# bjack205/rsLQR

Hardware: AMD Instinct MI355X
Metric: LQR solves/sec (nx=12,nu=4,N=256,batch=1024 per GPU) (higher is better)
Workload: dtype f64; 1 GPU; nx=12 nu=4 N=256 batch=1024 per GPU, fp64, factor+solve per step; parallelism=batch-sharded x1, no data-path collective, ranks_seen=1, flags=0, schedule=reduced-fused2

## Files before the change

include/ndlqr_hip.h:

```cpp
#ifndef NDLQR_HIP_H_
#define NDLQR_HIP_H_

#include <stddef.h>
#include <stdint.h>

#ifdef __cplusplus
extern "C" {
#endif

typedef struct NdlqrHipCtx NdlqrHipCtx;

int ndlqr_hip_device_count(void);
const char* ndlqr_hip_last_error(void);

NdlqrHipCtx* ndlqr_hip_create(int nstates, int ninputs, int nhorizon, int batch, int device);
#define NDLQR_CREATE_NO_PAD 1u
NdlqrHipCtx* ndlqr_hip_create_ex(int nstates, int ninputs, int nhorizon, int batch, int device, unsigned create_flags);
void ndlqr_hip_destroy(NdlqrHipCtx* ctx);
int ndlqr_hip_set_flags(NdlqrHipCtx* ctx, unsigned flags);
unsigned ndlqr_hip_get_flags(const NdlqrHipCtx* ctx);
int ndlqr_hip_set_stream(NdlqrHipCtx* ctx, void* hip_stream);
void* ndlqr_hip_get_stream(NdlqrHipCtx* ctx);

int ndlqr_hip_upload_inputs(NdlqrHipCtx* ctx, int p0, int count, const double* AB,
// ... 73 lines not shown
int ndlqr_hip_solve_polished_adjoint(NdlqrHipCtx* ctx, const double* g, int max_steps, int* steps, int* status);
int ndlqr_hip_download_polish_codes(NdlqrHipCtx* ctx, unsigned char* codes);
int ndlqr_hip_solve_multi_rhs(NdlqrHipCtx* ctx, int nrhs, const double* q, const double* r, const double* d,
                              const double* x0, double* soln);
int ndlqr_hip_solve_multi_rhs_slices(NdlqrHipCtx* ctx, int nrhs, const double* q, const double* r, const double* d,
                                     const double* x0, int knot0, int nknots, unsigned blocks, double* out);

int ndlqr_hip_step_async(NdlqrHipCtx* ctx, const double* q, const double* r, const double* d, const double* x0,
                         double* soln);
int ndlqr_hip_synchronize_previous(NdlqrHipCtx* ctx);
int ndlqr_hip_set_step_selection(NdlqrHipCtx* ctx, int knot0, int nknots, unsigned blocks);
int ndlqr_hip_solve_slices_async(NdlqrHipCtx* ctx, int knot0, int nknots, unsigned blocks, double* out);
int ndlqr_hip_download_selection(NdlqrHipCtx* ctx, int knot0, int nknots, unsigned blocks, double* out);
int ndlqr_hip_time_shard_top_doubles(NdlqrHipCtx* ctx, int G);
int ndlqr_hip_time_shard_factor(NdlqrHipCtx* ctx, int g, int G);
int ndlqr_hip_time_shard_export(NdlqrHipCtx* ctx, int G, double* buf);
int ndlqr_hip_time_shard_import(NdlqrHipCtx* ctx, int G, const double* buf);
int ndlqr_hip_time_shard_finish(NdlqrHipCtx* ctx, int g, int G);
void* ndlqr_hip_host_alloc(size_t bytes);
void ndlqr_hip_host_free(void* p);
void* ndlqr_hip_device_alloc(size_t bytes);
void ndlqr_hip_device_free(void* p);
int ndlqr_hip_copy(void* dst, const void* src, size_t bytes);

int ndlqr_hip_download_solutions(NdlqrHipCtx* ctx, int p0, int count, double* soln);
int ndlqr_hip_download_rhs_blocks(NdlqrHipCtx* ctx, int p, double* z_full);
int ndlqr_hip_download_factors(NdlqrHipCtx* ctx, int p, double* fact);
int ndlqr_hip_factors_valid(const NdlqrHipCtx* ctx);
int ndlqr_hip_pack_solutions_device(NdlqrHipCtx* ctx, double* dst);
int ndlqr_hip_kkt_residual(NdlqrHipCtx* ctx, double* res, double* bnorm);
int ndlqr_hip_cholesky_failures(NdlqrHipCtx* ctx);
const char* ndlqr_hip_schedule(const NdlqrHipCtx* ctx);
int ndlqr_hip_compact_level1(const NdlqrHipCtx* ctx);

int ndlqr_hip_profile_slots(NdlqrHipCtx* ctx);
int ndlqr_hip_profile_get(NdlqrHipCtx* ctx, int slot, char* name, int name_cap, double* total_ms,
                          int* launches);
int ndlqr_hip_profile_reset(NdlqrHipCtx* ctx);

int ndlqr_hip_gemm(int tA, int tB, int m, int n, int k, double alpha, const double* A, int lda,
                   const double* B, int ldb, double beta, double* C, int ldc);
int ndlqr_hip_potrf_lower(int n, double* A, int lda);
int ndlqr_hip_potrs_lower(int n, int nrhs, const double* L, int ldl, double* B, int ldb);
int ndlqr_hip_trsv_lower(int n, int nrhs, const double* L, int ldl, double* B, int ldb, int transposed);

#ifdef __cplusplus
}
#endif
#endif
```

rslqr_amd/api.py:

```python
import ctypes as C
import os
import re

import numpy as np

from . import build as _build

FLAG_STRICT_FP = 1
FLAG_GENERIC = 2
FLAG_PROFILE = 4
FLAG_KEEP_FACT = 8
FLAG_KEEP_RECORDS = 16
SOLN_LAMBDA, SOLN_STATE, SOLN_INPUT, SOLN_ONLY = 1, 2, 4, 8
GRAD_A, GRAD_B, GRAD_Q, GRAD_R, GRAD_q, GRAD_r, GRAD_d, GRAD_x0 = 1, 2, 4, 8, 16, 32, 64, 128
GRAD_NAMES = ("A", "B", "Q", "R", "q", "r", "d", "x0")

ERR_INVALID = -1
ERR_NO_DEVICE = -2
ERR_NOT_SPD = -3

dp = C.POINTER(C.c_double)


class Matrix(C.Structure):
# ... 254 lines not shown
    proto("ndlqr_BatchKktResidualVector", ci, vp, dp)
    proto("ndlqr_hip_refine_phase_ms", ci, vp, dp)
    proto("ndlqr_BatchDeviceContext", vp, vp)
    proto("ndlqr_BatchSetBounds", ci, vp, C.c_uint, dp, dp, dp, dp)
    proto("ndlqr_SolveBatchBoxConstrained", ci, vp, C.POINTER(NdLqrBoxSettingsFull), C.POINTER(ci), C.POINTER(ci))
    proto("ndlqr_CopyBatchBoundMultipliers", ci, vp, dp, dp)
    proto("ndlqr_CopyBatchBoxPenalties", ci, vp, dp)
    proto("ndlqr_CopyBatchBoxResiduals", ci, vp, dp)
    proto("ndlqr_CopyBatchBoxAdjointResiduals", ci, vp, dp)
    proto("ndlqr_BatchSetInfeasibilityDetection", ci, vp, ci, cd)
    proto("ndlqr_CopyBatchInfeasibilityCertificate", ci, vp, dp, dp, dp)
    proto("ndlqr_CopyBatchInfeasibilityMeasures", ci, vp, dp, C.POINTER(ci))
    proto("ndlqr_BatchSetBoxAcceleration", ci, vp, ci, cd, cd)
    proto("ndlqr_CopyBatchBoxAcceleration", ci, vp, C.POINTER(ci), C.POINTER(ci), dp, C.POINTER(ci))
    proto("ndlqr_SolveBatchBoxAdjoint", ci, vp, dp, C.POINTER(NdLqrBoxSettingsFull), C.POINTER(ci), C.POINTER(ci))
    proto("ndlqr_BatchBoundGradients", ci, vp, C.c_uint, dp, dp, dp, dp)
    proto("ndlqr_PolishBatchBoxConstrained", ci, vp, C.POINTER(NdLqrPolishSettings), C.POINTER(ci), C.POINTER(ci))
    proto("ndlqr_hip_download_polish_codes", ci, vp, C.POINTER(C.c_ubyte))
    proto("ndlqr_SolveBatchPolishedAdjoint", ci, vp, dp, C.POINTER(NdLqrPolishSettings), C.POINTER(ci), C.POINTER(ci))
    proto("ndlqr_hip_factor_count", C.c_ulonglong, vp)
    proto("ndlqr_hip_set_stream", ci, vp, vp)
    proto("ndlqr_hip_get_stream", vp, vp)
    proto("ndlqr_hip_profile_slots", ci, vp)
    proto("ndlqr_hip_profile_get", ci, vp, ci, C.c_char_p, ci, dp, C.POINTER(ci))
    proto("ndlqr_hip_profile_reset", ci, vp)
    proto("ndlqr_hip_device_pointers", ci, vp, C.POINTER(vp))
    proto("ndlqr_hip_staged_io", ci, vp, C.POINTER(dp), C.POINTER(dp), C.POINTER(dp), C.POINTER(dp))
    proto("ndlqr_hip_download_rhs_blocks", ci, vp, ci, dp)
    proto("ndlqr_hip_upload_inputs", ci, vp, ci, ci, dp, dp, dp)
    proto("ndlqr_hip_factors_valid", ci, vp)
    proto("ndlqr_hip_schedule", C.c_char_p, vp)
    if hasattr(L, "ndlqr_hip_compact_level1"):
        proto("ndlqr_hip_compact_level1", C.c_int, vp)
    proto("ndlqr_hip_set_pipeline_depth", ci, vp, ci)
    proto("ndlqr_hip_pipeline_depth", ci, vp)
    proto("ndlqr_hip_pack_solutions_device", ci, vp, vp)
    proto("ndlqr_hip_gemm", ci, ci, ci, ci, ci, ci, cd, dp, ci, dp, ci, cd, dp, ci)
    proto("ndlqr_hip_potrf_lower", ci, ci, dp, ci)
    proto("ndlqr_hip_potrs_lower", ci, ci, ci, dp, ci, dp, ci)
    _LIB = L
    return L


def pinned_empty(shape):
    import weakref
    count = int(np.prod(shape))
    L = lib()
    ptr = L.ndlqr_HostAlloc(max(count, 1) * 8)
    if not ptr:
        raise MemoryError("ndlqr_HostAlloc(%d bytes) failed" % (count * 8))
    buf = (C.c_double * max(count, 1)).from_address(ptr)
    arr = np.ctypeslib.as_array(buf)[:count].reshape(shape)
    weakref.finalize(buf, L.ndlqr_HostFree, C.c_void_p(ptr))
    return arr


class DeviceArray:

    def __init__(self, shape):
        import weakref
        self.shape = tuple(int(s) for s in (shape if isinstance(shape, (tuple, list)) else (shape,)))
        self.size = int(np.prod(self.shape))
        L = lib()
        self.ptr = L.ndlqr_DeviceAlloc(max(self.size, 1) * 8)
        if not self.ptr:
            raise MemoryError("ndlqr_DeviceAlloc(%d bytes) failed" % (self.size * 8))
# ... 707 lines not shown
        err = self.L.ndlqr_hip_upload_inputs(self.ctx, 0, self.batch, _ptr(AB), _ptr(QR), _ptr(rhs))
        if err:
            raise RuntimeError("ndlqr_hip_upload_inputs failed: %d" % err)

    def factors(self, p):
        if self.N & (self.N - 1):
            raise RuntimeError("ndlqr_CopyBatchFactors: not available for a padded horizon (horizon %d is no power of two)"
                               % self.N)
        K = int(np.log2(self.N))
        out = np.zeros(self.N * K * (2 * self.n + self.m) * self.n)
        err = self.L.ndlqr_CopyBatchFactors(self.h, p, _ptr(out))
        if err:
            raise RuntimeError("ndlqr_CopyBatchFactors failed: %d" % err)
        return out

    def cholesky_failures(self):
        return self.L.ndlqr_BatchCholeskyFailures(self.h)

    def profile(self):
        out = {}
        for slot in range(self.L.ndlqr_hip_profile_slots(self.ctx)):
            name = C.create_string_buffer(64)
            ms, cnt = C.c_double(0), C.c_int(0)
            self.L.ndlqr_hip_profile_get(self.ctx, slot, name, 64, C.byref(ms), C.byref(cnt))
            out[name.value.decode()] = (ms.value, cnt.value)
        return out

    def schedule(self):
        return self.L.ndlqr_hip_schedule(self.ctx).decode()

    def compact_level1(self):
        return hasattr(self.L, "ndlqr_hip_compact_level1") and bool(self.L.ndlqr_hip_compact_level1(self.ctx))

    def set_pipeline_depth(self, depth):
        return self.L.ndlqr_hip_set_pipeline_depth(self.ctx, depth)

    def pipeline_depth(self):
        return self.L.ndlqr_hip_pipeline_depth(self.ctx)

    def profile_reset(self):
        self.L.ndlqr_hip_profile_reset(self.ctx)
```

rslqr_amd/csrc/hip_context.hpp:

```cpp
#pragma once
#include <hip/hip_runtime.h>

#include <cstdio>
#include <cstdlib>
#include <cstring>
#include <initializer_list>
#include <string>
#include <utility>
#include <vector>

#include "ndlqr.h"
#include "ndlqr_hip.h"

#include "kernels_common.hpp"

#pragma GCC visibility push(hidden)
int ndlqr_hip_fail(const char* what, hipError_t e);
struct NdlqrHipCtx;
int ndlqr_hip_ensure_F(NdlqrHipCtx* c);
#pragma GCC visibility pop
#define HIP_TRY(expr)                                                  \
  do {                                                                 \
    hipError_t e_ = (expr);                                            \
    if (e_ != hipSuccess) return ndlqr_hip_fail(#expr, e_);            \
  } while (0)

constexpr size_t kLdsMax = 160 * 1024;
constexpr size_t kLdsDefaultDynamic = 64 * 1024;
template <class Kernel>
static inline hipError_t allow_dynamic_lds(Kernel* kernel, size_t lds) {
  if (lds <= kLdsDefaultDynamic) return hipSuccess;
  return hipFuncSetAttribute(reinterpret_cast<const void*>(kernel), hipFuncAttributeMaxDynamicSharedMemorySize, (int)lds);
}


enum { SLOT_LEAF = 0, SLOT_SEP, SLOT_SCHUR, SLOT_BOUNDARY, SLOT_APPLY, SLOT_BOTTOM, SLOT_UPPER, SLOT_TOP, SLOT_COUNT };

struct PendingEvent {
  int slot;
  hipEvent_t start, stop;
};

enum class Family { None, Small, GenericReduced, GenericKnot };

struct KeptState {
  Family family = Family::None;
  bool time_shard = false;
  bool rec_complete = false;
  bool rec_compact = false;
  bool fact_valid = false;
  const char* schedule = "none";
  bool rec1_compact = false;
  void forget_factorisation() { rec_complete = fact_valid = false; }
};

struct CapturedChain {
  hipGraphExec_t exec = nullptr;
  unsigned flags = 0;
  hipStream_t stream = nullptr;
  unsigned apply = 0;
  void reset() {
    if (exec) (void)hipGraphExecDestroy(exec);
    exec = nullptr;
  }
};

struct KnotSlice {
  int knot0 = 0, nknots = 0;
  unsigned blocks = 7u;
  bool valid(int N, unsigned allowed) const {
    return knot0 >= 0 && nknots > 0 && knot0 + nknots <= N && (blocks & 7u) && !(blocks & ~allowed);
  }
  size_t width(const ndlqr::Dims& u) const {
    return ((blocks & 1u) ? u.n : 0) + ((blocks & 2u) ? u.n : 0) + ((blocks & 4u) ? u.m : 0);
  }
  size_t doubles(const ndlqr::Dims& u) const { return nknots > 0 ? width(u) * nknots : (size_t)u.rows * u.N - u.m; }
};

#pragma GCC visibility push(hidden)

template <class T, bool PINNED>
class OwnedBuf {
  T* p_ = nullptr;
  size_t n_ = 0;

// ... 37 lines not shown

static inline size_t doubles_QR(const ndlqr::Dims& d) { return (size_t)d.batch * d.N * d.w; }
static inline size_t doubles_z(const ndlqr::Dims& d) { return (size_t)d.batch * d.N * d.rows; }
static inline size_t doubles_F(const ndlqr::Dims& d) { return (size_t)d.batch * d.K * d.N * d.fb; }
static inline hipError_t first_error(std::initializer_list<hipError_t> list) {
  for (const hipError_t e : list) if (e != hipSuccess) return e;
  return hipSuccess;
}

struct BufferSet {
  DevBuf<double> rec;
  DevBuf<double> red;
  DevBuf<double> ytop;
  DevBuf<double> z;
  DevBuf<double> rhs;
  DevBuf<double> xfer;
  DevBuf<int> tree_cnt;
  PinnedBuf<int> h_fail;
  hipStream_t stream = nullptr;
  hipEvent_t ev_start = nullptr, ev_stop = nullptr;
  unsigned long long rhs_gen[4] = {};
  CapturedChain graph;
  bool ready = false;
  hipError_t ensure_xfer(const ndlqr::Dims& u) { return xfer.ensure((size_t)u.batch * u.N * u.rows + (size_t)u.batch * u.n); }
};


struct DevKnobs {
  int rowbcast = -1;
  int tree = -1;
  int backsub_cols = -1;
  int fuse2 = -1;
  int compact1 = -1;
  int pipeline = 2;
  bool no_top = false;
  int top_levels = 3;
  bool no_mfma = false;
  int sep_threads = 0;
  int mult_threads = 0;
  bool no_reduced_generic = false;
  bool no_pad = false;
  bool alt_priority_set = false;
  int alt_priority = 0;
};

struct AdjointState {
  DevBuf<double> rhs, z;
  DevBuf<double> save;
  unsigned long long gen = 0;
  hipError_t ensure_save(const ndlqr::Dims& d) { return save.ensure(2 * (size_t)d.batch * d.N * d.n); }
  hipError_t ensure(const ndlqr::Dims& d, hipStream_t st) {
    return first_error({rhs.ensure(doubles_z(d)), z.ensure_zeroed(doubles_z(d), st), ensure_save(d)});
  }
};

struct BoxState {
  DevBuf<double> lo, hi, v, y, z, qr_save, rhs[2], resid, rho;
  DevBuf<unsigned char> mask;
  DevBuf<int> status, iters, word;
  PinnedBuf<int> h_word;
  bool shared = false, have_bounds = false, have_vy = false;
  size_t bstride = 0;
  bool fact = false;
  bool rho_uniform = false;
  double rho_value = 0.0;
  unsigned flags = 0;
// ... 296 lines not shown
```

rslqr_amd/csrc/kernels_bottom_reduced.hpp:

```cpp
#pragma once
#include "kernels_dpp.hpp"
#include "kernels_small.hpp"

namespace ndlqr {

typedef double acc4_t __attribute__((ext_vector_type(4)));

template <int NX>
struct McPitch {
  static constexpr int SP = 18, WP = 17;
};

template <int NX, class Hook>
__device__ __forceinline__ void factor_tail_mc(const int lane, const acc4_t& c, const double (&ra)[(NX + 3) / 4],
                                               const double (&rb)[(NX + 3) / 4], const double* Wm, acc4_t& X0,
                                               acc4_t& X1, Hook hook) {
  constexpr int KS = (NX + 3) / 4, WP = McPitch<NX>::WP;
  int lane_o = lane;
  asm volatile("" : "+v"(lane_o));
  const int li = lane_o & 15, lk = lane_o >> 4;
  double wt[KS], wa[KS], b0[KS];
#pragma unroll
  for (int q = 0; q < KS; ++q) {
    wt[q] = Wm[(4 * q + lk) * WP + li];
// ... 181 lines not shown
  for (int g = 0; g < 4; ++g) {
    buf[P::SCR_A + (lk + 4 * g) * SP + li] = cA[g];
    buf[P::SCR_B + (lk + 4 * g) * SP + li] = cB[g];
  }
  wave_lds_sync();
  const double* tile = buf + (lk < 2 ? P::SCR_A : P::SCR_B);
  double acc[NX];
  if constexpr (NX % 2 == 0) {
#pragma unroll
    for (int j = 0; j < NX; j += 2) {
      const double2 t = *reinterpret_cast<const double2*>(&tile[ri * SP + j]);
      acc[j] = t.x; acc[j + 1] = t.y;
    }
  } else {
#pragma unroll
    for (int j = 0; j < NX; ++j) acc[j] = tile[ri * SP + j];
  }
  if (h == NX) {
#pragma unroll
    for (int k = 0; k < NX; ++k) w[k] = tile[k * SP + NX];
  }
  const bool bad = rb_chol_inv<NX, false>(li, acc, w);
  wave_lds_sync();
  {
    const int x = lk >> 1;
    double* ydst = buf + (h <= NX ? P::tile(x, 0) + h : P::tile(x, 1) + (h <= 2 * NX ? h - NX - 1 : YP - 1));
#pragma unroll
    for (int k = 0; k < NX; ++k) ydst[k * YP] = w[k];
    if constexpr (4 * KS > NX) {
#pragma unroll
      for (int e0 = 0; e0 < (4 * KS - NX) * YP; e0 += 16) {
        const int e = e0 + li;
        if (e < (4 * KS - NX) * YP) buf[P::tile(x, lk & 1) + NX * YP + e] = 0.0;
      }
    }
  }
  if ((lk & 1) == 0 && li < NX) {
    double* lr = (lk == 0 ? lrecA : lrecB) + li * (li + 1) / 2;
#pragma unroll
    for (int c = 0; c < NX; ++c)
      if (c <= li) lr[c] = acc[c];
  }
  wave_lds_sync();
  return bad;
}

template <int NX, bool N00, bool N01, bool N10, bool N11>
__device__ __forceinline__ void gram_mc(const double (&R0)[(NX + 3) / 4], const double (&R1)[(NX + 3) / 4],
                                        const acc4_t& X0, const acc4_t& X1, acc4_t& g00, acc4_t& g01, acc4_t& g10,
                                        acc4_t& g11) {
  constexpr int KS = (NX + 3) / 4;
  const acc4_t zero = {0.0, 0.0, 0.0, 0.0};
  g00 = zero; g01 = zero; g10 = zero; g11 = zero;
#pragma unroll
  for (int q = 0; q < KS; ++q) {
    if constexpr (N00) g00 = __builtin_amdgcn_mfma_f64_16x16x4f64(R0[q], X0[q], g00, 0, 0, 0);
    if constexpr (N01) g01 = __builtin_amdgcn_mfma_f64_16x16x4f64(R0[q], X1[q], g01, 0, 0, 0);
    if constexpr (N10) g10 = __builtin_amdgcn_mfma_f64_16x16x4f64(R1[q], X0[q], g10, 0, 0, 0);
    if constexpr (N11) g11 = __builtin_amdgcn_mfma_f64_16x16x4f64(R1[q], X1[q], g11, 0, 0, 0);
  }
}

template <int NX> __device__ __forceinline__ constexpr bool rows_all(int g) { return 4 * g + 3 < NX; }
template <int NX> __device__ __forceinline__ constexpr bool rows_none(int g) { return 4 * g >= NX; }

template <int NX>
// ... 300 lines not shown
  constexpr int NN = NX * NX, KS = P::KS;
  const int N = d.N, T = 8, s = base + 3;
  const bool hasA = base > 0, hasB = base + T < N, leftchild = (base & T) == 0;
  const int li = lane & 15, lk = lane >> 4;
  double y0[KS], y1[KS];
  acc4_t Z0 = {0.0, 0.0, 0.0, 0.0}, Z1 = {0.0, 0.0, 0.0, 0.0};
#pragma unroll
  for (int q = 0; q < KS; ++q) {
    y0[q] = buf[P::Y0 + (4 * q + lk) * P::YP + li];
    y1[q] = buf[P::Y1 + (4 * q + lk) * P::YP + li];
    Z0[q] = y0[q]; Z1[q] = y1[q];
  }
  if (gram) {
    const RedSlot<NX> sa = red_slot<NX>(red, d, b, hasA ? base - 1 : s);
    const RedSlot<NX> sb = red_slot<NX>(red, d, b, hasB ? base + T - 1 : s);
    acc4_t g00, g01, g11, unused;
    gram_mc<NX, true, true, false, true>(y0, y1, Z0, Z1, g00, g01, unused, g11);
    const acc4_t zero = {0.0, 0.0, 0.0, 0.0};
    push_mc<NX>(lane, hasA, hasB, leftchild, sa, sb, g00, g01, g11, zero, zero, zero, AddAtomic(), StorePlain());
  } else {
    double wt[KS];
#pragma unroll
    for (int q = 0; q < KS; ++q) wt[q] = buf[P::W + (4 * q + lk) * P::WP + li];
    acc4_t X0 = {0.0, 0.0, 0.0, 0.0}, X1 = {0.0, 0.0, 0.0, 0.0};
#pragma unroll
    for (int q = 0; q < KS; ++q) {
      X0 = __builtin_amdgcn_mfma_f64_16x16x4f64(wt[q], y0[q], X0, 0, 0, 0);
      X1 = __builtin_amdgcn_mfma_f64_16x16x4f64(wt[q], y1[q], X1, 0, 0, 0);
    }
    store_record_mc<NX>(rec + ((size_t)b * N + s) * (2 * NN + NX), lane, hasA, hasB, X0, X1);
  }
}

template <int NX, int NU, bool TREE, bool REDIRECT, bool C1 = false>
__device__ __forceinline__ void bottom_group_mc(const Dims& d, const int k0, const int b, const int lane,
                                                const double* __restrict__ AB, const double* __restrict__ QR,
                                                const double* __restrict__ rhs, double* red, double* __restrict__ rec,
                                                double* F, int* __restrict__ info, const int store_l, const int compact0,
                                                ReducedLds<NX, NU>& lds, double* slotA, double* slotB,
                                                const bool with_m = false, acc4_t* c_m = nullptr);
template <int NX, int NU, bool C1 = false>
__global__ __launch_bounds__(128) __attribute__((amdgpu_waves_per_eu(4))) void bottom8_reduced_mc(
    Dims d, const double* __restrict__ AB, const double* __restrict__ QR, const double* __restrict__ rhs, double* red,
    double* __restrict__ rec, int* __restrict__ info) {
  __shared__ ReducedLds<NX, NU> lds[2];
  __shared__ __attribute__((aligned(16))) double mslot[RedSlot<NX>::SIZE];
  const int wave = __builtin_amdgcn_readfirstlane(threadIdx.x >> 6), b = blockIdx.y;
  const int kw = (blockIdx.x + d.xoff) * 8;
  int lane = threadIdx.x & 63;
  for (int e = threadIdx.x; e < RedSlot<NX>::SIZE; e += 128) mslot[e] = 0.0;
  __syncthreads();
  acc4_t c_m = {0.0, 0.0, 0.0, 0.0};
  bottom_group_mc<NX, NU, false, true, C1>(d, kw + 4 * wave, b, lane, AB, QR, rhs, red, rec, nullptr, info, 0, 1, lds[wave],
                                       wave == 1 ? mslot : nullptr, wave == 0 ? mslot : nullptr, wave == 0, &c_m);
  asm volatile("s_waitcnt vmcnt(0)" ::: "memory");
  __syncthreads();
  asm volatile("" : "+v"(lane));
  if (wave == 0) reduced_eliminate_pass_mc<NX, NU>(d, kw, b, lane, c_m, mslot, info, lds[0].buf);
  __syncthreads();
  reduced_eliminate_tail_mc<NX, NU>(d, kw, b, lane, wave == 0, red, rec, lds[0].buf);
}

template <int NX>
__device__ __forceinline__ void backsub_top_body(const Dims& d, const int b, const int t,
                                                 const double* __restrict__ recs, double* __restrict__ ytop,
                                                 double* ytop_lds, const int bp = -1, const double* zsep = nullptr);
template <int NX, int NU>
__global__ __launch_bounds__(256) __attribute__((amdgpu_waves_per_eu(4))) void reduced_top_mc(Dims d, const int l0, const double* __restrict__ AB,
                                                      const double* __restrict__ QR, const double* __restrict__ rhs,
                                                      double* red, double* __restrict__ rec, double* F,
                                                      int* __restrict__ info, const int store_l,
                                                      double* __restrict__ ytop) {
  __shared__ ReducedLds<NX, NU, false> lds[4];
  const int wave = __builtin_amdgcn_readfirstlane(threadIdx.x >> 6), b = blockIdx.x;
  for (int l = l0, s0 = 0; l < d.K;) {
    int lane = threadIdx.x & 63;
    asm volatile("" : "+v"(lane));
    const int cnt = d.N >> (l + 1);
    if (wave + s0 < cnt)
      reduced_separator_mc<NX, NU, true>(d, l, (wave + s0) * (2 << l), b, lane, AB, QR, rhs, red, rec, F, info, store_l,
                                         lds[wave]);
    s0 += 4;
    if (s0 < cnt) continue;
    s0 = 0;
    ++l;
    asm volatile("s_waitcnt vmcnt(0)" ::: "memory");
    __syncthreads();
  }
  if (ytop) backsub_top_body<NX>(d, b, threadIdx.x, rec, ytop, reinterpret_cast<double*>(&lds[0]), -1, nullptr);
}

template <int NX, int NU, bool TREE, bool REDIRECT, bool C1>
__device__ __forceinline__ void bottom_group_mc(const Dims& d, const int k0, const int b, const int lane,
                                                const double* __restrict__ AB, const double* __restrict__ QR,
                                                const double* __restrict__ rhs, double* red, double* __restrict__ rec,
                                                double* F, int* __restrict__ info, const int store_l, const int compact0,
                                                ReducedLds<NX, NU>& lds, double* slotA, double* slotB,
                                                const bool with_m, acc4_t* c_m) {
  constexpr int W = NX + NU, ROWS = 2 * NX + NU, NN = NX * NX, KSN = (NX + 3) / 4;
  constexpr int REC = 2 * NN + NX;
  constexpr int WP = ReducedLds<NX, NU>::WP;
  double* abs_ = lds.buf;
  double* rq = lds.rq;
  double* rh = lds.rh;
  const int N = d.N;
  const int li = lane & 15, lk = lane >> 4;
  const int ri = li < NX ? li : NX - 1;
  const bool hasA = k0 > 0, hasB = k0 + 4 < N;
  SEG_INIT();

  {
    const double* abm = AB + ((size_t)b * N + k0) * NX * W;
    const double* q0 = QR + ((size_t)b * N + k0) * W;
    const double* r0 = rhs + ((size_t)b * N + k0) * ROWS;
    constexpr int NQ = 4 * W, IQ = (NQ + 63) / 64, NR = 4 * ROWS, IR = (NR + 63) / 64;
    double qv[IQ], rv[IR];
#pragma unroll
    for (int it = 0; it < IQ; ++it) { const int e = lane + 64 * it; qv[it] = q0[e < NQ ? e : NQ - 1]; }
#pragma unroll
    for (int it = 0; it < IR; ++it) { const int e = lane + 64 * it; rv[it] = r0[e < NR ? e : NR - 1]; }
    if constexpr (W % 2 == 0) {
      constexpr int NA = 4 * NX * W / 2, IA = (NA + 63) / 64;
      double2 t[IA];
#pragma unroll
      for (int it = 0; it < IA; ++it) {
        const int e = lane + 64 * it;
        t[it] = reinterpret_cast<const double2*>(abm)[e < NA ? e : NA - 1];
      }
#pragma unroll
      for (int it = 0; it < IA; ++it) {
        const int e = lane + 64 * it, ec = e < NA ? e : NA - 1, row = ec / (W / 2), c2 = ec - row * (W / 2);
// ... 96 lines not shown
        y1[q] = Y1[(4 * q + lk) * PY::YP + li];
        Z0[q] = y0[q]; Z1[q] = y1[q];
      }
      if (x == 0) hook_s0(y0, y1, Z0, Z1); else hook_s2(y0, y1, Z0, Z1);
    }
    SEG(35);
  } else {
  double ra0[KSN], rb0[KSN], ra2[KSN], rb2[KSN];
#pragma unroll
  for (int q = 0; q < KSN; ++q) {
    const int kq = 4 * q + lk, i = kq < NX ? kq : NX - 1;
    const double a0 = abs_[i * WP + ri], b0 = abs_[(NX + ri) * WP + i];
    const double a2 = abs_[(2 * NX + i) * WP + ri], b2 = abs_[(3 * NX + ri) * WP + i];
    const double s0 = rq[ri], s1 = rq[W + i], s2 = rq[2 * W + ri], s3 = rq[3 * W + i];
    ra0[q] = hasA ? -a0 * s0 : 0.0;
    rb0[q] = -b0 * s1;
    ra2[q] = -a2 * s2;
    rb2[q] = hasB ? -b2 * s3 : 0.0;
  }
  wave_lds_sync();
  SEG(21);

  using Pair = McPairLayout<NX>;
  if (chol_pair_mc<NX>(lane, c_s0, c_s2, lds.buf, store_l ? Fblk(F, d, b, 0, k0 + 1) : nullptr,
                       store_l ? Fblk(F, d, b, 0, k0 + 3) : nullptr) &&
      (lane == 0 || lane == 32))
    flag_failure(info, d, b);
  SEG(30);
  factor_tail_mc<NX>(lane, c_s0, ra0, rb0, lds.buf + Pair::W_A, X0, X1, hook_s0);
  store_record_mc<NX>(myrec, lane, hasA, true, X0, X1);
  factor_tail_mc<NX>(lane, c_s2, ra2, rb2, lds.buf + Pair::W_B, X0, X1, hook_s2);
  store_record_mc<NX>(myrec + 2 * REC, lane, true, hasB, X0, X1);
  SEG(35);
  }
  double wcol[NX];
  {
    constexpr int TP = 17;
    static_assert(2 * 16 * TP <= ReducedLds<NX, NU>::NBUF, "both coupling tiles fit the buffer");
    double* ta = lds.buf;
    double* tb = lds.buf + 16 * TP;
    wave_lds_sync();
#pragma unroll
    for (int g = 0; g < 4; ++g) {
      ta[(lk + 4 * g) * TP + li] = -ca_t[g];
      tb[(lk + 4 * g) * TP + li] = -cb_t[g];
    }
    wave_lds_sync();
    const int h = lane & 31;
    const bool is_a = h < NX, is_b = h > NX && h <= 2 * NX;
    const double* src = is_a ? ta + h : tb + (is_b ? h - NX - 1 : 0);
#pragma unroll
    for (int k = 0; k < NX; ++k) wcol[k] = src[k * TP];
    wave_lds_sync();
  }
  const bool leftchild = (k0 & 4) == 0;
  RedSlot<NX> sa = red_slot<NX>(red, d, b, hasA ? k0 - 1 : 3);
  RedSlot<NX> sb = red_slot<NX>(red, d, b, hasB ? k0 + 3 : 3);
  if constexpr (REDIRECT) {
    if (slotA) sa.p = slotA;
    if (slotB) sb.p = slotB;
  }
  if constexpr (C1) {
    static_assert(!TREE, "the tree schedule keeps full records");
    if (chol_pair_y_mc<NX>(lane, c_t, c_t, lds.buf, wcol, myrec + REC, myrec + REC) && lane == 0) flag_failure(info, d, b);
    SEG(34);
    using PY = McPairYLayout<NX>;
// ... 74 lines not shown
```

rslqr_amd/csrc/launch_small.hpp:

```cpp
#pragma once
#include "hip_context.hpp"
#include "kernels_leaf.hpp"
#include "kernels_small.hpp"
#include "kernels_bottom_reduced.hpp"
#include "kernels_rowbcast.hpp"

constexpr int kBottomLevels = 2;

struct SmallPlan {
  bool strict, keep;
  bool lean;
  int store_l;
  bool reduced;
  bool tree;
  bool compact;
  bool rowbcast;
  bool fuse2;
  bool compact1;
  int level0;
  int ltop;
  int top_l0;
  bool top_sweeps;
  size_t top_lds;
  const char* schedule;
  bool rec_complete, rec_compact;
  bool needs_F;
};

template <int NX, int NU>
constexpr bool kRbBacksubFits = 8 * (2 * NX + NU) <= 256;

static inline unsigned apply_grid(const NdlqrHipCtx* c, const ndlqr::Dims& d) {
  return (unsigned)(c->apply_nblk > 0 ? c->apply_nblk : d.N / 8);
}
static inline ndlqr::Dims apply_dims(const NdlqrHipCtx* c, const ndlqr::Dims& d) {
  ndlqr::Dims da = d;
  if (c->apply_nblk > 0) da.xoff += c->apply_blk0;
  return da;
}

template <int NX, int NU>
constexpr bool kCompact1Fits = ndlqr::P1OnMatrixCores<NX, NU>::value && NX >= 9 && NX + NU <= 16;

template <int NX, int NU, bool MULTI, class... Args>
static void launch_rb_backsub(const NdlqrHipCtx* c, const dim3 grid, hipStream_t stream, const bool compact1,
                              const Args&... args) {
  if constexpr (NX + NU <= 16) {
    if constexpr (kCompact1Fits<NX, NU> && !MULTI) {
      if (compact1) {
        hipLaunchKernelGGL((ndlqr::rb_backsub<NX, NU, false, true, true>), grid, dim3(ndlqr::kRbBacksubColsThreads), 0, stream,
                           args...);
        return;
      }
    }
    if (c->knobs.backsub_cols != 0) {
      hipLaunchKernelGGL((ndlqr::rb_backsub<NX, NU, MULTI, true>), grid, dim3(ndlqr::kRbBacksubColsThreads), 0, stream, args...);
      return;
    }
  }
  hipLaunchKernelGGL((ndlqr::rb_backsub<NX, NU, MULTI, false>), grid, dim3(256), 0, stream, args...);
}

template <int NX, int NU>
static SmallPlan plan_small(const NdlqrHipCtx* c, const bool strict, const bool keep) {
  const ndlqr::Dims& d = c->d;
  const BufferSet& s = c->set[0];
  SmallPlan p = {};
  p.strict = strict;
  p.keep = keep;
  p.lean = !strict && !keep && (d.K + 4) * NX <= 256;
  p.store_l = (c->flags & NDLQR_FLAG_KEEP_RECORDS) ? 1 : 0;
  p.rec_complete = !strict && (keep || (p.lean && p.store_l));
  p.level0 = p.ltop = p.top_l0 = d.K;
  p.schedule = p.lean ? "knot-lean" : (strict ? "knot-strict" : "knot-keep");
  if constexpr (ndlqr::P1OnMatrixCores<NX, NU>::value) {
    if (p.lean && s.red) {
      p.reduced = true;
      p.tree = s.tree_cnt && (c->knobs.tree == 1 || (c->knobs.tree < 0 && (size_t)d.batch * (d.N >> 2) <= 2048));
      p.top_lds = sizeof(double) * (size_t)(d.N >> 3) * NX;
      p.compact = !p.tree && d.N >= 16 && kRbBacksubFits<NX, NU> && p.top_lds * (p.store_l ? 4 : 1) <= kLdsMax;
      if (p.compact && p.store_l) p.store_l = 2;
      p.rec_compact = p.compact && p.store_l == 2;
      p.rowbcast = p.compact && !p.store_l && NX <= 16 && NX + NU <= 16 && (c->knobs.rowbcast == 1 || (c->knobs.rowbcast < 0 && NX <= 8));
      p.fuse2 = !p.rowbcast && p.compact && !p.store_l && (c->knobs.fuse2 > 0 || (c->knobs.fuse2 < 0 && NX == 12 && NU == 4));
      p.compact1 = kCompact1Fits<NX, NU> && p.compact && !p.store_l && !p.rowbcast && c->knobs.backsub_cols != 0 &&
                   (c->knobs.compact1 > 0 ||
                    (c->knobs.compact1 < 0 && ((NX == 12 && NU == 4 && p.fuse2) || (NX == 10 && NU == 4))));
      p.schedule = p.tree ? "reduced-tree"
                   : !p.compact ? "reduced-records"
                   : p.store_l ? "reduced-compact-records" : (p.fuse2 ? "reduced-fused2" : "reduced");
      if (!p.tree) {
        const int top_levels = d.K - c->knobs.top_levels >= 3 ? c->knobs.top_levels : 3;
        p.level0 = p.fuse2 ? 3 : 2;
        p.ltop = (d.K >= 5 && !c->knobs.no_top) ? d.K - top_levels : d.K;
        p.top_l0 = (p.fuse2 && p.ltop < 3) ? 3 : p.ltop;
        p.top_sweeps = p.ltop < d.K && p.compact && p.top_lds <= 4 * sizeof(ndlqr::ReducedLds<NX, NU, false>);
      }
    }
  }
  p.needs_F = !(p.reduced && p.store_l != 1);
  return p;
}

template <int NX, int NU, bool STRICT, bool KEEP>
static int launch_small(NdlqrHipCtx* c, const SmallPlan& plan) {
  const ndlqr::Dims& d = c->d;
  BufferSet& s = c->set[c->cur];
  using Sh = ndlqr::SchurShape<NX, NU>;
  constexpr int JB = kBottomLevels;
  const bool lean = plan.lean;
  const int store_l = plan.store_l;
  if constexpr (!STRICT && !KEEP && ndlqr::P1OnMatrixCores<NX, NU>::value) {
    if (plan.reduced) {
      {
        ScopedSlot t(c, SLOT_BOTTOM);
        if (plan.rowbcast) {
          if constexpr (NX <= 16 && NX + NU <= 16)
            hipLaunchKernelGGL((ndlqr::rb_bottom<NX, NU>), dim3(d.N >> 4, d.batch), dim3(64), 0, s.stream, d, c->AB,
                               c->QR, s.rhs, s.red, s.rec, c->info);
        } else if (plan.fuse2) {
          bool done = false;
          if constexpr (kCompact1Fits<NX, NU>) {
            if (plan.compact1) {
              hipLaunchKernelGGL((ndlqr::bottom8_reduced_mc<NX, NU, true>), dim3(d.N >> 3, d.batch), dim3(128), 0, s.stream, d,
                                 c->AB, c->QR, s.rhs, s.red, s.rec, c->info);
              done = true;
            }
          }
          if (!done)
            hipLaunchKernelGGL((ndlqr::bottom8_reduced_mc<NX, NU>), dim3(d.N >> 3, d.batch), dim3(128), 0, s.stream, d,
                               c->AB, c->QR, s.rhs, s.red, s.rec, c->info);
        } else if (plan.tree)
          hipLaunchKernelGGL((ndlqr::bottom_reduced_mc<NX, NU, true>), dim3(d.N >> 2, d.batch), dim3(64), 0, s.stream,
                             d, c->AB, c->QR, s.rhs, s.red, s.rec, c->F, c->info, store_l, s.tree_cnt, 0);
        else if (plan.compact) {
          bool done = false;
          if constexpr (kCompact1Fits<NX, NU>) {
            if (plan.compact1) {
              hipLaunchKernelGGL((ndlqr::bottom_reduced_mc<NX, NU, false, true, true>), dim3(d.N >> 2, d.batch), dim3(64), 0,
                                 s.stream, d, c->AB, c->QR, s.rhs, s.red, s.rec, c->F, c->info, store_l, nullptr, 1);
              done = true;
            }
          }
          if (!done)
            hipLaunchKernelGGL((ndlqr::bottom_reduced_mc<NX, NU, false, true>), dim3(d.N >> 2, d.batch), dim3(64), 0, s.stream,
                               d, c->AB, c->QR, s.rhs, s.red, s.rec, c->F, c->info, store_l, nullptr, 1);
        } else
          hipLaunchKernelGGL((ndlqr::bottom_reduced_mc<NX, NU, false>), dim3(d.N >> 2, d.batch), dim3(64), 0, s.stream,
                             d, c->AB, c->QR, s.rhs, s.red, s.rec, c->F, c->info, store_l, nullptr, 0);
      }
      for (int l = plan.level0; l < plan.ltop; ++l) {
        ScopedSlot t(c, SLOT_UPPER);
        hipLaunchKernelGGL((ndlqr::reduced_level_mc<NX, NU>), dim3(d.N >> (l + 1), d.batch), dim3(64), 0, s.stream,
                           d, l, c->AB, c->QR, s.rhs, s.red, s.rec, c->F, c->info, store_l);
      }
      if (plan.ltop < d.K) {
// ... 191 lines not shown
```

rslqr_amd/csrc/ndlqr_hip.hip:

```cpp
#include "hip_host.hpp"
#include "kernels_generic.hpp"
#include "kernels_mfma.hpp"
#include "launch_reduced.hpp"
#include "kernels_reduced_solve.hpp"
#include "launch_small.hpp"


static thread_local std::string g_last_error = "";

const char* ndlqr_hip_last_error(void) { return g_last_error.c_str(); }

int ndlqr_hip_fail(const char* what, hipError_t e) {
  g_last_error = std::string(what) + ": " + hipGetErrorString(e);
  fprintf(stderr, "ndlqr_hip: %s\n", g_last_error.c_str());
  if (e == hipErrorInvalidConfiguration || e == hipErrorInvalidValue) return NDLQR_ERR_INVALID;
  return NDLQR_ERR_NO_DEVICE;
}
int fail(const char* what, hipError_t e) { return ndlqr_hip_fail(what, e); }
int refuse(const std::string& msg) {
  g_last_error = msg;
  fprintf(stderr, "ndlqr_hip: %s\n", g_last_error.c_str());
  return NDLQR_ERR_INVALID;
}

// ... 42 lines not shown
  for (const SmallInstance* s : kSmallInstances)
    if (s->nx == nstates && s->nu == ninputs) return true;
  return false;
}

static void pick_pad_instance(int nstates, int ninputs, int* pn, int* pm) {
  long best = -1;
  for (const SmallInstance* si : kSmallInstances) {
    if (si->nx < nstates || si->nu < ninputs || si->nx < 6) continue;
    const long cost = (long)si->nx * si->nx * (si->nx + si->nu);
    if (best < 0 || cost < best) { best = cost; *pn = si->nx; *pm = si->nu; }
  }
}

static const SmallInstance* find_small(const ndlqr::Dims& d) {
  for (const SmallInstance* s : kSmallInstances)
    if (s->nx == d.n && s->nu == d.m) return s;
  return nullptr;
}

static size_t bytes_z(const ndlqr::Dims& d) { return sizeof(double) * doubles_z(d); }
static size_t bytes_F(const ndlqr::Dims& d) { return sizeof(double) * doubles_F(d); }

static DevKnobs read_knobs() {
  DevKnobs k;
  const auto num = [](const char* name, int* v) { if (getenv(name)) *v = atoi(getenv(name)); };
  const auto onoff = [](const char* name, int* v) { if (getenv(name)) *v = atoi(getenv(name)) != 0 ? 1 : 0; };
  num("NDLQR_PIPELINE", &k.pipeline);
  onoff("NDLQR_TREE", &k.tree);
  onoff("NDLQR_ROWBCAST", &k.rowbcast);
  onoff("NDLQR_FUSE2", &k.fuse2);
  onoff("NDLQR_BACKSUB_COLS", &k.backsub_cols);
  onoff("NDLQR_COMPACT1", &k.compact1);
  k.no_mfma = getenv("NDLQR_NO_MFMA") != nullptr;
  k.no_top = getenv("NDLQR_NO_TOP") != nullptr;
  num("NDLQR_TOP_LEVELS", &k.top_levels);
  if (k.top_levels < 3 || k.top_levels > 5) k.top_levels = 3;
  num("NDLQR_SEP_THREADS", &k.sep_threads);
  num("NDLQR_MULT_THREADS", &k.mult_threads);
  k.no_reduced_generic = getenv("NDLQR_DEV_NO_REDUCED_GENERIC") != nullptr;
  k.no_pad = getenv("NDLQR_NO_PAD") != nullptr;
  k.alt_priority_set = getenv("NDLQR_ALT_PRIORITY") != nullptr;
  num("NDLQR_ALT_PRIORITY", &k.alt_priority);
  return k;
}

static bool alloc_set(NdlqrHipCtx* c, BufferSet& s, bool slots) {
  const ndlqr::Dims& d = c->d;
  hipError_t e = first_error({hipEventCreate(&s.ev_start), hipEventCreate(&s.ev_stop), s.rec.ensure((size_t)d.batch * d.N * (2 * d.n * d.n + d.n)),
                              s.rhs.ensure(doubles_z(d)), s.h_fail.ensure_zeroed(1)});
  if (e == hipSuccess && slots) {
    const size_t slot_doubles = ((size_t)d.n * (d.n + 1) + 2 * (size_t)d.n * d.n + 2 * d.n + 15) / 16 * 16;
    e = first_error({s.red.ensure_zeroed((size_t)d.batch * (d.N / 4) * slot_doubles, s.stream),
                     s.ytop.ensure((size_t)d.batch * (d.N / 8) * d.n),
                     s.tree_cnt.ensure_zeroed((size_t)d.batch * (d.N / 4), s.stream)});
  }
  return e == hipSuccess && s.z.ensure_zeroed(doubles_z(d), s.stream) == hipSuccess;
}

NdlqrHipCtx* ndlqr_hip_create(int nstates, int ninputs, int nhorizon, int batch, int device) {
  return ndlqr_hip_create_ex(nstates, ninputs, nhorizon, batch, device, 0u);
}

NdlqrHipCtx* ndlqr_hip_create_ex(int nstates, int ninputs, int nhorizon, int batch, int device, unsigned create_flags) {
  if (nstates <= 0 || ninputs <= 0 || batch <= 0 || nhorizon < 2 || nhorizon > (1 << 24)) {
    g_last_error = "invalid dimensions";
// ... 541 lines not shown
    const int work = d.N * d.rows;
    hipLaunchKernelGGL(ndlqr::backsub_states_generic, dim3((work + 255) / 256, d.batch), dim3(256), 0, s.stream, d,
                       c->AB, c->QR, s.rhs, s.z);
  }
  return NDLQR_OK;
}

static const SmallInstance* pick_small(const NdlqrHipCtx* c) {
  const ndlqr::Dims& d = c->d;
  if (c->flags & NDLQR_FLAG_GENERIC) return nullptr;
  const SmallInstance* inst = find_small(d);
  if (!inst || d.N < inst->kpb || d.K < 3) return nullptr;
  return inst;
}

static const SmallInstance* kept_instance(const NdlqrHipCtx* c) {
  return c->kept.family == Family::Small ? find_small(c->d) : nullptr;
}

static SolvePlan plan_solve(const NdlqrHipCtx* c) {
  const ndlqr::Dims& d = c->d;
  SolvePlan p = {};
  p.strict = (c->flags & NDLQR_FLAG_STRICT_FP) != 0;
  p.keep = (c->flags & NDLQR_FLAG_KEEP_FACT) != 0;
  p.inst = pick_small(c);
  if (p.inst) {
    p.family = Family::Small;
    p.small = p.inst->plan(c, p.strict, p.keep);
    p.needs_F = p.small.needs_F;
    p.kept.schedule = p.small.schedule;
    p.kept.rec_complete = p.small.rec_complete;
    p.kept.rec_compact = p.small.rec_compact;
    p.kept.rec1_compact = p.small.compact1;
  } else if ((p.red = plan_reduced_generic(c)).ok) {
    p.family = Family::GenericReduced;
    p.needs_red_generic = true;
    p.kept.schedule = p.red.keep ? "generic-reduced-records" : "generic-reduced";
    p.kept.rec_complete = p.red.keep;
  } else {
    p.family = Family::GenericKnot;
    p.rec_as_factors = (c->flags & NDLQR_FLAG_KEEP_RECORDS) && !p.strict;
    p.lean = !p.strict && !p.keep && !p.rec_as_factors;
    p.needs_F = true;
    p.sep = plan_generic_sep(c, p.strict);
    if (p.sep.scratch)
      p.sep_scratch_bytes = sizeof(double) * ((size_t)d.n * (d.n + 1) + (size_t)d.n * (2 * d.n + 1)) * (size_t)d.batch *
                            (d.N / 2 > 0 ? d.N / 2 : 1);
    p.kept.schedule = p.lean ? "generic-lean" : (p.strict ? "generic-strict" : "generic-keep");
  }
  p.kept.family = p.family;
  p.kept.fact_valid = p.keep || p.rec_as_factors || ((c->flags & NDLQR_FLAG_GENERIC) && p.strict);
  p.may_pipeline = !p.needs_F && !(c->flags & (NDLQR_FLAG_PROFILE | NDLQR_FLAG_KEEP_RECORDS | NDLQR_FLAG_KEEP_FACT));
  return p;
}

static int enqueue_solve(NdlqrHipCtx* c, const SolvePlan& plan) {
  BufferSet& s = c->set[c->cur];
  int err = NDLQR_OK;
  switch (plan.family) {
    case Family::Small: err = plan.inst->solve(c, plan.small); break;
    case Family::GenericReduced: err = launch_reduced_generic(c, plan.red); break;
    default: err = plan.strict ? launch_generic<true>(c, plan) : launch_generic<false>(c, plan); break;
  }
  if (!err) HIP_TRY(hipMemcpyAsync(s.h_fail, c->info + c->d.batch, sizeof(int), hipMemcpyDeviceToHost, s.stream));
  return err;
}
// ... 762 lines not shown
  const size_t chunk = (8u << 20) / sizeof(double);
  if (total <= chunk / 8) {
    HIP_TRY(hipMemcpyAsync(soln, s.xfer, sizeof(double) * total, hipMemcpyDeviceToHost, st));
    HIP_TRY(hipStreamSynchronize(st));
    return NDLQR_OK;
  }
  for (int i = 0; i < 2; ++i)
    HIP_TRY(c->h_stage[i].ensure(chunk));
  hipEvent_t done[2] = {take_event(c), take_event(c)};
  const size_t nchunks = (total + chunk - 1) / chunk;
  hipError_t e = hipSuccess;
  for (size_t i = 0; i <= nchunks && e == hipSuccess; ++i) {
    if (i < nchunks) {
      const size_t off = i * chunk, len = total - off < chunk ? total - off : chunk;
      e = hipMemcpyAsync(c->h_stage[i & 1], s.xfer + off, sizeof(double) * len, hipMemcpyDeviceToHost, st);
      if (e == hipSuccess) e = hipEventRecord(done[i & 1], st);
    }
    if (i > 0 && e == hipSuccess) {
      const size_t off = (i - 1) * chunk, len = total - off < chunk ? total - off : chunk;
      e = hipEventSynchronize(done[(i - 1) & 1]);
      if (e == hipSuccess) memcpy(soln + off, c->h_stage[(i - 1) & 1], sizeof(double) * len);
    }
  }
  c->event_pool.push_back(done[0]);
  c->event_pool.push_back(done[1]);
  if (e != hipSuccess) return fail("ndlqr_hip_download_solutions", e);
  return NDLQR_OK;
}

const char* ndlqr_hip_schedule(const NdlqrHipCtx* c) { return c ? c->kept.schedule : "none"; }

int ndlqr_hip_compact_level1(const NdlqrHipCtx* c) { return c && c->kept.rec1_compact ? 1 : 0; }

int ndlqr_hip_factors_valid(const NdlqrHipCtx* c) { return c && c->kept.fact_valid ? 1 : 0; }

int ndlqr_hip_pack_solutions_device(NdlqrHipCtx* c, double* dst) {
  if (!c || !dst) return NDLQR_ERR_INVALID;
  if (c->z_partial || c->z_invalid) return need_full_solution(c, "ndlqr_hip_pack_solutions_device");
  const ndlqr::Dims& d = c->d;
  HIP_TRY(hipSetDevice(c->device));
  HIP_TRY(launch_pack(c->du, d, KnotSlice(), c->set[c->latest].z, dst, c->set[c->latest].stream, d.batch));
  if (c->cost.dense && !c->cost.mapped(c->soln_gen)) HIP_TRY(cost_map_back(c, dst, 0, d.batch, c->set[c->latest].stream));
  return NDLQR_OK;
}

int ndlqr_hip_kkt_residual(NdlqrHipCtx* c, double* res, double* bnorm) {
  if (!c || !res) return NDLQR_ERR_INVALID;
  if (const int cerr = need_diagonal_cost(c, "ndlqr_hip_kkt_residual")) return cerr;
  if (c->z_partial || c->z_invalid) return need_full_solution(c, "ndlqr_hip_kkt_residual");
  const ndlqr::Dims& d = c->d;
  BufferSet& s = c->set[c->cur];
  HIP_TRY(hipSetDevice(c->device));
  HIP_TRY(c->kkt_out.ensure(2 * (size_t)d.batch));
  double* out = c->kkt_out;
  HIP_TRY(sync_all(c));
  hipLaunchKernelGGL(ndlqr::kkt_residual_generic, dim3(d.batch), dim3(256), 0, s.stream, d, c->AB, c->QR, s.rhs,
                     c->set[c->latest].z, out);
  hipError_t e = hipGetLastError();
  if (e == hipSuccess) e = hipMemcpyAsync(res, out, sizeof(double) * d.batch, hipMemcpyDeviceToHost, s.stream);
  if (e == hipSuccess && bnorm)
    e = hipMemcpyAsync(bnorm, out + d.batch, sizeof(double) * d.batch, hipMemcpyDeviceToHost, s.stream);
  if (e == hipSuccess) e = hipStreamSynchronize(s.stream);
  if (e != hipSuccess) return fail("ndlqr_hip_kkt_residual", e);
  return NDLQR_OK;
}

// ... 78 lines not shown
```

Baseline: 1.984 million solves/s.

## Pair level-1 separator factorizations across both wavefronts in fused bottom kernel

Adds a paired level-1 pass to the fused bottom8 reduced kernel. Each wavefront hands its separator tile and couplings through LDS, and wavefront 0 factors both separators' Cholesky/Y in one call, using half-wave lanes for each. The shared tail then builds the Gram matrices and pushes them upward. This aims to raise lane utilisation in the level-1 Cholesky, which previously ran per wavefront at low lane occupancy for NX=12. The cost is extra block-wide syncs, an idle second wavefront during the paired factor, and more code paths. It is enabled by default for NX=12, NU=4.

```diff
diff --git a/include/ndlqr_hip.h b/include/ndlqr_hip.h
--- a/include/ndlqr_hip.h
+++ b/include/ndlqr_hip.h
@@ -129,6 +129,7 @@
 int ndlqr_hip_cholesky_failures(NdlqrHipCtx* ctx);
 const char* ndlqr_hip_schedule(const NdlqrHipCtx* ctx);
 int ndlqr_hip_compact_level1(const NdlqrHipCtx* ctx);
+int ndlqr_hip_level1_paired(const NdlqrHipCtx* ctx);
 
 int ndlqr_hip_profile_slots(NdlqrHipCtx* ctx);
 int ndlqr_hip_profile_get(NdlqrHipCtx* ctx, int slot, char* name, int name_cap, double* total_ms,
diff --git a/rslqr_amd/api.py b/rslqr_amd/api.py
--- a/rslqr_amd/api.py
+++ b/rslqr_amd/api.py
@@ -310,6 +310,8 @@
     proto("ndlqr_hip_schedule", C.c_char_p, vp)
     if hasattr(L, "ndlqr_hip_compact_level1"):
         proto("ndlqr_hip_compact_level1", C.c_int, vp)
+    if hasattr(L, "ndlqr_hip_level1_paired"):
+        proto("ndlqr_hip_level1_paired", C.c_int, vp)
     proto("ndlqr_hip_set_pipeline_depth", ci, vp, ci)
     proto("ndlqr_hip_pipeline_depth", ci, vp)
     proto("ndlqr_hip_pack_solutions_device", ci, vp, vp)
@@ -1083,6 +1085,9 @@
     def compact_level1(self):
         return hasattr(self.L, "ndlqr_hip_compact_level1") and bool(self.L.ndlqr_hip_compact_level1(self.ctx))
 
+    def level1_paired(self):
+        return hasattr(self.L, "ndlqr_hip_level1_paired") and bool(self.L.ndlqr_hip_level1_paired(self.ctx))
+
     def set_pipeline_depth(self, depth):
         return self.L.ndlqr_hip_set_pipeline_depth(self.ctx, depth)
 
diff --git a/rslqr_amd/csrc/hip_context.hpp b/rslqr_amd/csrc/hip_context.hpp
--- a/rslqr_amd/csrc/hip_context.hpp
+++ b/rslqr_amd/csrc/hip_context.hpp
@@ -51,6 +51,7 @@
   bool fact_valid = false;
   const char* schedule = "none";
   bool rec1_compact = false;
+  bool level1_paired = false;
   void forget_factorisation() { rec_complete = fact_valid = false; }
 };
 
@@ -154,6 +155,7 @@
   int backsub_cols = -1;
   int fuse2 = -1;
   int compact1 = -1;
+  int pair1 = -1;
   int pipeline = 2;
   bool no_top = false;
   int top_levels = 3;
diff --git a/rslqr_amd/csrc/kernels_bottom_reduced.hpp b/rslqr_amd/csrc/kernels_bottom_reduced.hpp
--- a/rslqr_amd/csrc/kernels_bottom_reduced.hpp
+++ b/rslqr_amd/csrc/kernels_bottom_reduced.hpp
@@ -237,6 +237,80 @@
       for (int e0 = 0; e0 < (4 * KS - NX) * YP; e0 += 16) {
         const int e = e0 + li;
         if (e < (4 * KS - NX) * YP) buf[P::tile(x, lk & 1) + NX * YP + e] = 0.0;
+      }
+    }
+  }
+  if ((lk & 1) == 0 && li < NX) {
+    double* lr = (lk == 0 ? lrecA : lrecB) + li * (li + 1) / 2;
+#pragma unroll
+    for (int c = 0; c < NX; ++c)
+      if (c <= li) lr[c] = acc[c];
+  }
+  wave_lds_sync();
+  return bad;
+}
+
+template <int NX>
+struct McPair1Layout {
+  static constexpr int SP = McPitch<NX>::SP, TP = 17;
+  static constexpr int SCR = 0, TA = 16 * SP, TB = TA + 16 * TP, SIZE = TB + 16 * TP;
+};
+template <int NX>
+__device__ __forceinline__ void pair1_exchange_mc(const int lane_in, const acc4_t& c_t, const acc4_t& ca_t,
+                                                  const acc4_t& cb_t, double* buf) {
+  using X = McPair1Layout<NX>;
+  int lane = lane_in;
+  asm volatile("" : "+v"(lane));
+  const int li = lane & 15, lk = lane >> 4;
+  wave_lds_sync();
+#pragma unroll
+  for (int g = 0; g < 4; ++g) {
+    buf[X::SCR + (lk + 4 * g) * X::SP + li] = c_t[g];
+    buf[X::TA + (lk + 4 * g) * X::TP + li] = li == NX ? c_t[g] : -ca_t[g];
+    buf[X::TB + (lk + 4 * g) * X::TP + li] = -cb_t[g];
+  }
+}
+template <int NX>
+__device__ __forceinline__ bool chol_pair1_y_mc(const int lane_in, double* bufA, double* bufB, double* lrecA,
+                                                double* lrecB) {
+  using P = McPairYLayout<NX>;
+  using X = McPair1Layout<NX>;
+  constexpr int SP = P::SP, YP = P::YP, KS = P::KS;
+  static_assert(2 * P::TILE <= X::SIZE, "the Y tiles of one separator lie inside what its wavefront wrote");
+  int lane = lane_in;
+  asm volatile("" : "+v"(lane));
+  const int li = lane & 15, lk = lane >> 4, h = lane & 31;
+  const int ri = li < NX ? li : NX - 1;
+  double* buf = lk < 2 ? bufA : bufB;
+  const double* tile = buf + X::SCR;
+  double acc[NX], w[NX];
+  if constexpr (NX % 2 == 0) {
+#pragma unroll
+    for (int j = 0; j < NX; j += 2) {
+      const double2 t = *reinterpret_cast<const double2*>(&tile[ri * SP + j]);
+      acc[j] = t.x; acc[j + 1] = t.y;
+    }
+  } else {
+#pragma unroll
+    for (int j = 0; j < NX; ++j) acc[j] = tile[ri * SP + j];
+  }
+  {
+    const bool is_b = h > NX && h <= 2 * NX;
+    const double* src = buf + (h <= NX ? X::TA + h : X::TB + (is_b ? h - NX - 1 : 0));
+#pragma unroll
+    for (int k = 0; k < NX; ++k) w[k] = src[k * X::TP];
+  }
+  const bool bad = rb_chol_inv<NX, false>(li, acc, w);
+  wave_lds_sync();
+  {
+    double* ydst = buf + (h <= NX ? P::tile(0, 0) + h : P::tile(0, 1) + (h <= 2 * NX ? h - NX - 1 : YP - 1));
+#pragma unroll
+    for (int k = 0; k < NX; ++k) ydst[k * YP] = w[k];
+    if constexpr (4 * KS > NX) {
+#pragma unroll
+      for (int e0 = 0; e0 < (4 * KS - NX) * YP; e0 += 16) {
+        const int e = e0 + li;
+        if (e < (4 * KS - NX) * YP) buf[P::tile(0, lk & 1) + NX * YP + e] = 0.0;
       }
     }
   }
@@ -603,14 +677,42 @@
   }
 }
 
-template <int NX, int NU, bool TREE, bool REDIRECT, bool C1 = false>
+struct Pair1Hand { acc4_t c_t, ca_t, cb_t, park_a, park_b11; };
+template <int NX, int NU>
+__device__ __forceinline__ void pair1_tail_mc(const Dims& d, const int k0, const int b, const int lane_in, double* red,
+                                              const double* buf, const Pair1Hand& hd, double* slotA, double* slotB) {
+  using PY = McPairYLayout<NX>;
+  constexpr int KSN = (NX + 3) / 4;
+  int lane = lane_in;
+  asm volatile("" : "+v"(lane));
+  const int li = lane & 15, lk = lane >> 4;
+  const bool hasA = k0 > 0, hasB = k0 + 4 < d.N, leftchild = (k0 & 4) == 0;
+  RedSlot<NX> sa = red_slot<NX>(red, d, b, hasA ? k0 - 1 : 3);
+  RedSlot<NX> sb = red_slot<NX>(red, d, b, hasB ? k0 + 3 : 3);
+  if (slotA) sa.p = slotA;
+  if (slotB) sb.p = slotB;
+  double y0[KSN], y1[KSN];
+  acc4_t Z0 = {0.0, 0.0, 0.0, 0.0}, Z1 = {0.0, 0.0, 0.0, 0.0};
+#pragma unroll
+  for (int q = 0; q < KSN; ++q) {
+    y0[q] = buf[PY::tile(0, 0) + (4 * q + lk) * PY::YP + li];
+    y1[q] = buf[PY::tile(0, 1) + (4 * q + lk) * PY::YP + li];
+    Z0[q] = y0[q]; Z1[q] = y1[q];
+  }
+  acc4_t g00, g01, g11, unused;
+  gram_mc<NX, true, true, false, true>(y0, y1, Z0, Z1, g00, g01, unused, g11);
+  push_mc<NX>(lane, hasA, hasB, leftchild, sa, sb, g00, g01, g11, hd.park_a, hd.cb_t, hd.park_b11, StorePlain(), StorePlain());
+}
+
+template <int NX, int NU, bool TREE, bool REDIRECT, bool C1 = false, bool P1 = false>
 __device__ __forceinline__ void bottom_group_mc(const Dims& d, const int k0, const int b, const int lane,
                                                 const double* __restrict__ AB, const double* __restrict__ QR,
                                                 const double* __restrict__ rhs, double* red, double* __restrict__ rec,
                                                 double* F, int* __restrict__ info, const int store_l, const int compact0,
                                                 ReducedLds<NX, NU>& lds, double* slotA, double* slotB,
-                                                const bool with_m = false, acc4_t* c_m = nullptr);
-template <int NX, int NU, bool C1 = false>
+                                                const bool with_m = false, acc4_t* c_m = nullptr,
+                                                Pair1Hand* hand = nullptr);
+template <int NX, int NU, bool C1 = false, bool P1 = false>
 __global__ __launch_bounds__(128) __attribute__((amdgpu_waves_per_eu(4))) void bottom8_reduced_mc(
     Dims d, const double* __restrict__ AB, const double* __restrict__ QR, const double* __restrict__ rhs, double* red,
     double* __restrict__ rec, int* __restrict__ info) {
@@ -622,8 +724,27 @@
   for (int e = threadIdx.x; e < RedSlot<NX>::SIZE; e += 128) mslot[e] = 0.0;
   __syncthreads();
   acc4_t c_m = {0.0, 0.0, 0.0, 0.0};
+  if constexpr (P1) {
+    static_assert(C1, "the paired pass is the Y-only pass of compact level-1 records");
+    static_assert(McPair1Layout<NX>::SIZE <= ReducedLds<NX, NU>::NBUF, "tile and couplings of t fit the wavefront's buffer");
+    Pair1Hand hd;
+    bottom_group_mc<NX, NU, false, true, true, true>(d, kw + 4 * wave, b, lane, AB, QR, rhs, red, rec, nullptr, info, 0, 1,
+                                                     lds[wave], nullptr, nullptr, wave == 0, &c_m, &hd);
+    pair1_exchange_mc<NX>(lane, hd.c_t, hd.ca_t, hd.cb_t, lds[wave].buf);
+    __syncthreads();
+    if (wave == 0) {
+      double* rec_t0 = rec + ((size_t)b * d.N + kw + 1) * (2 * NX * NX + NX);
+      if (chol_pair1_y_mc<NX>(lane, lds[0].buf, lds[1].buf, rec_t0, rec_t0 + 4 * (2 * NX * NX + NX)) &&
+          (lane == 0 || lane == 32))
+        flag_failure(info, d, b);
+    }
+    __syncthreads();
+    pair1_tail_mc<NX, NU>(d, kw + 4 * wave, b, lane, red, lds[wave].buf, hd, wave == 1 ? mslot : nullptr,
+                          wave == 0 ? mslot : nullptr);
+  } else {
   bottom_group_mc<NX, NU, false, true, C1>(d, kw + 4 * wave, b, lane, AB, QR, rhs, red, rec, nullptr, info, 0, 1, lds[wave],
                                        wave == 1 ? mslot : nullptr, wave == 0 ? mslot : nullptr, wave == 0, &c_m);
+  }
   asm volatile("s_waitcnt vmcnt(0)" ::: "memory");
   __syncthreads();
   asm volatile("" : "+v"(lane));
@@ -661,13 +782,14 @@
   if (ytop) backsub_top_body<NX>(d, b, threadIdx.x, rec, ytop, reinterpret_cast<double*>(&lds[0]), -1, nullptr);
 }
 
-template <int NX, int NU, bool TREE, bool REDIRECT, bool C1>
+template <int NX, int NU, bool TREE, bool REDIRECT, bool C1, bool P1>
 __device__ __forceinline__ void bottom_group_mc(const Dims& d, const int k0, const int b, const int lane,
                                                 const double* __restrict__ AB, const double* __restrict__ QR,
                                                 const double* __restrict__ rhs, double* red, double* __restrict__ rec,
                                                 double* F, int* __restrict__ info, const int store_l, const int compact0,
                                                 ReducedLds<NX, NU>& lds, double* slotA, double* slotB,
-                                                const bool with_m, acc4_t* c_m) {
+                                                const bool with_m, acc4_t* c_m, Pair1Hand* hand) {
+  static_assert(!P1 || (C1 && REDIRECT && !TREE), "the paired level-1 pass: the fused bottom launch with compact level-1 records");
   constexpr int W = NX + NU, ROWS = 2 * NX + NU, NN = NX * NX, KSN = (NX + 3) / 4;
   constexpr int REC = 2 * NN + NX;
   constexpr int WP = ReducedLds<NX, NU>::WP;
@@ -830,6 +952,10 @@
   factor_tail_mc<NX>(lane, c_s2, ra2, rb2, lds.buf + Pair::W_B, X0, X1, hook_s2);
   store_record_mc<NX>(myrec + 2 * REC, lane, true, hasB, X0, X1);
   SEG(35);
+  }
+  if constexpr (P1) {
+    hand->c_t = c_t; hand->ca_t = ca_t; hand->cb_t = cb_t; hand->park_a = park_a; hand->park_b11 = park_b11;
+    return;
   }
   double wcol[NX];
   {
diff --git a/rslqr_amd/csrc/launch_small.hpp b/rslqr_amd/csrc/launch_small.hpp
--- a/rslqr_amd/csrc/launch_small.hpp
+++ b/rslqr_amd/csrc/launch_small.hpp
@@ -17,6 +17,7 @@
   bool rowbcast;
   bool fuse2;
   bool compact1;
+  bool pair1;
   int level0;
   int ltop;
   int top_l0;
@@ -41,6 +42,9 @@
 
 template <int NX, int NU>
 constexpr bool kCompact1Fits = ndlqr::P1OnMatrixCores<NX, NU>::value && NX >= 9 && NX + NU <= 16;
+
+template <int NX, int NU>
+constexpr bool kPair1Fits = kCompact1Fits<NX, NU> && ndlqr::McPair1Layout<NX>::SIZE <= ndlqr::ReducedLds<NX, NU>::NBUF;
 
 template <int NX, int NU, bool MULTI, class... Args>
 static void launch_rb_backsub(const NdlqrHipCtx* c, const dim3 grid, hipStream_t stream, const bool compact1,
@@ -86,6 +90,8 @@
       p.compact1 = kCompact1Fits<NX, NU> && p.compact && !p.store_l && !p.rowbcast && c->knobs.backsub_cols != 0 &&
                    (c->knobs.compact1 > 0 ||
                     (c->knobs.compact1 < 0 && ((NX == 12 && NU == 4 && p.fuse2) || (NX == 10 && NU == 4))));
+      p.pair1 = kPair1Fits<NX, NU> && p.fuse2 && p.compact1 &&
+                (c->knobs.pair1 > 0 || (c->knobs.pair1 < 0 && NX == 12 && NU == 4));
       p.schedule = p.tree ? "reduced-tree"
                    : !p.compact ? "reduced-records"
                    : p.store_l ? "reduced-compact-records" : (p.fuse2 ? "reduced-fused2" : "reduced");
@@ -120,8 +126,15 @@
                                c->QR, s.rhs, s.red, s.rec, c->info);
         } else if (plan.fuse2) {
           bool done = false;
+          if constexpr (kPair1Fits<NX, NU>) {
+            if (plan.pair1) {
+              hipLaunchKernelGGL((ndlqr::bottom8_reduced_mc<NX, NU, true, true>), dim3(d.N >> 3, d.batch), dim3(128), 0, s.stream,
+                                 d, c->AB, c->QR, s.rhs, s.red, s.rec, c->info);
+              done = true;
+            }
+          }
           if constexpr (kCompact1Fits<NX, NU>) {
-            if (plan.compact1) {
+            if (!done && plan.compact1) {
               hipLaunchKernelGGL((ndlqr::bottom8_reduced_mc<NX, NU, true>), dim3(d.N >> 3, d.batch), dim3(128), 0, s.stream, d,
                                  c->AB, c->QR, s.rhs, s.red, s.rec, c->info);
               done = true;
diff --git a/rslqr_amd/csrc/ndlqr_hip.hip b/rslqr_amd/csrc/ndlqr_hip.hip
--- a/rslqr_amd/csrc/ndlqr_hip.hip
+++ b/rslqr_amd/csrc/ndlqr_hip.hip
@@ -98,6 +98,7 @@
   onoff("NDLQR_FUSE2", &k.fuse2);
   onoff("NDLQR_BACKSUB_COLS", &k.backsub_cols);
   onoff("NDLQR_COMPACT1", &k.compact1);
+  onoff("NDLQR_PAIR1", &k.pair1);
   k.no_mfma = getenv("NDLQR_NO_MFMA") != nullptr;
   k.no_top = getenv("NDLQR_NO_TOP") != nullptr;
   num("NDLQR_TOP_LEVELS", &k.top_levels);
@@ -705,6 +706,7 @@
     p.kept.rec_complete = p.small.rec_complete;
     p.kept.rec_compact = p.small.rec_compact;
     p.kept.rec1_compact = p.small.compact1;
+    p.kept.level1_paired = p.small.pair1;
   } else if ((p.red = plan_reduced_generic(c)).ok) {
     p.family = Family::GenericReduced;
     p.needs_red_generic = true;
@@ -1533,6 +1535,8 @@
 
 int ndlqr_hip_compact_level1(const NdlqrHipCtx* c) { return c && c->kept.rec1_compact ? 1 : 0; }
 
+int ndlqr_hip_level1_paired(const NdlqrHipCtx* c) { return c && c->kept.level1_paired ? 1 : 0; }
+
 int ndlqr_hip_factors_valid(const NdlqrHipCtx* c) { return c && c->kept.fact_valid ? 1 : 0; }
 
 int ndlqr_hip_pack_solutions_device(NdlqrHipCtx* c, double* dst) {
```

Result: faster. 2.025 million solves/s (median of 6 runs) (+2.0%).
